# Healthcare-Robotics/mr-gan

Hardware: NVIDIA B200
Metric: gan_train_step_pairs_per_sec (higher is better)
Workload: dtype f16

## Files before the change

### mr_gan_b200/csrc/common.cuh

```cuda
#pragma once
#include <cuda_fp16.h>
#include <cuda_runtime.h>
#include <stdint.h>

#define MRGAN_TID_Z 5

enum { ACT_NONE = 0, ACT_RELU = 1, ACT_SOFTPLUS = 2, ACT_LEAKY = 3 };
enum { EPI_FWD = 0, EPI_DX = 1, EPI_STORE = 2 };

struct FoldState {
  uint32_t key0, key1;
  int iterations;
  int it_net[2];
  int rng_step;
  float lr_t[2];
  int D, n_train, n_test;
  int ldx;
  const float* x_train;
  const int* y_train;
  const int* y_test;
  const int* idx[3];
  const float* stage_x;
  const int* stage_y;
  const float* stage_z;
// ... 164 lines not shown
```

### mr_gan_b200/csrc/kernels_simt.cuh

```cuda
#pragma once
#include "common.cuh"

__device__ __forceinline__ float4 ldg4(const float* p) { return __ldg(reinterpret_cast<const float4*>(p)); }

template <bool AT, bool BT>
__global__ void __launch_bounds__(256)
k_gemm_simt(const GemmDesc* __restrict__ descs, const FoldState* __restrict__ folds, int rows_override, AdamHyper hp) {
  const GemmDesc d = descs[blockIdx.z];
  int M = d.M, K = d.K;
  const int N = d.N;
  if (rows_override > 0) { if (AT) K = rows_override; else M = rows_override; }
  const int m0 = blockIdx.y * 64, n0 = blockIdx.x * 64;
  if (m0 >= M || n0 >= N) return;

  __shared__ __align__(16) float As[2][16][68];
  __shared__ __align__(16) float Bs[2][16][68];
  const int tid = threadIdx.x, tx = tid & 15, ty = tid >> 4;
  const float4 zero4 = make_float4(0.f, 0.f, 0.f, 0.f);

  auto load_a = [&](int k0) -> float4 {
    if (AT) {
      const int k = k0 + (tid >> 4), m = m0 + (tid & 15) * 4;
      return (k < K && m < d.lda) ? ldg4(d.A + (size_t)k * d.lda + m) : zero4;
    } else {
// ... 117 lines not shown
      if (m >= M) continue;
      float v = acc[i][j];
      if (d.act == ACT_RELU) v = fmaxf(v, 0.f);
      else if (d.act == ACT_SOFTPLUS) v = softplusf(v);
      else if (d.act == ACT_LEAKY) v = v > 0.f ? v : hp.alpha * v;
      if (d.C) d.C[(size_t)m * d.ldc + n] = v;
      if (d.C2) d.C2[(size_t)m * d.ldc2 + n] = mul ? v * nz[i] : v + d.sigma * nz[i];
    }
  }
}

template <int PG>
__global__ void __launch_bounds__(128)
k_prep(FoldState* __restrict__ folds, int fold_base, int mode, int from_stage, int t, int B, int nrows,
       int noise_dim, float sigma_in, AdamHyper hp, OperandMode om) {
  FoldState& fs = folds[fold_base + blockIdx.z];
  const int c = blockIdx.x * 128 + threadIdx.x;
  const uint32_t step = (uint32_t)fs.rng_step;
  const int D = fs.D;

  if (blockIdx.x == 0 && blockIdx.y == 0) {
    if (threadIdx.x == 0) {
      const int net = (mode == 1) ? 1 : 0;
      const int tt = (hp.shared_t ? fs.iterations : fs.it_net[net]) + 1;
      const double b1t = pow((double)hp.b1, (double)tt), b2t = pow((double)hp.b2, (double)tt);
      fs.lr_t[net] = (float)((double)hp.lr * sqrt(1.0 - b2t) / (1.0 - b1t));
    }
    if (mode != 1) {
      for (int r = threadIdx.x; r < (mode == 2 ? nrows : B); r += 128)
        fs.labels_cur[r] = from_stage ? fs.stage_y[r] : fs.y_train[fs.idx[0][(size_t)t * B + r]];
// ... 154 lines not shown
  float var = 0.f;
  for (int i = 0; i < BN_SLICES; ++i) var += red[1][i][cx];
  if (!ok) return;
  const float istd = rsqrtf(var / d.B + eps);
  if (sl == 0) d.istd[j] = istd;
  const float g = d.gamma[j], b = d.beta[j];
  for (int r = sl; r < d.B; r += BN_SLICES) {
    const float xh = (d.h1[(size_t)r * d.ld + j] - mu) * istd;
    d.xhat[(size_t)r * d.ld + j] = xh;
    const float u = fmaf(g, xh, b);
    put_operand(d.u + (size_t)r * d.ldu + j, u, om);
  }
}

__global__ void __launch_bounds__(1024) k_bn_bwd(const BnDesc* __restrict__ descs, OperandMode om) {
  __shared__ float red[2][BN_MAX_SLICES][BN_COLS];
  const BnDesc d = descs[blockIdx.z];
  const int BN_SLICES = blockDim.x / BN_COLS;
  const int cx = threadIdx.x & (BN_COLS - 1), sl = threadIdx.x / BN_COLS;
  const int j = blockIdx.x * BN_COLS + cx;
  const bool ok = j < d.W;
  const float ginv = (om.mode == 2) ? 1.0f / om.gscale : 1.0f;
  float p1 = 0.f, p2 = 0.f;
  if (ok) for (int r = sl; r < d.B; r += BN_SLICES) {
    const float du = d.du[(size_t)r * d.ld + j] * ginv;
    p1 += du;
    p2 = fmaf(du, d.xhat[(size_t)r * d.ld + j], p2);
  }
  red[0][sl][cx] = p1; red[1][sl][cx] = p2;
  __syncthreads();
// ... 522 lines not shown
```

### mr_gan_b200/csrc/kernels_tc.cuh

```cuda
#pragma once
#include <cuda.h>
#include "common.cuh"

enum { HEAD_NONE = 0, HEAD_DISC = 1, HEAD_FM = 2, HEAD_BN = 3 };

struct alignas(64) TcOp {
  CUtensorMap mapA, mapB;
  GemmDesc g;
  int ME, NE, KE;
  int bn;
  int net;
  int ws_stride;
  float* ws;
  int esz;
  int head;
  int stats_stride;
  const void* hd;
  float* stats;
};

#define TC_KBLK 32
#define TC_SPIN_LIMIT (1ll << 31)

#ifdef MRGAN_PHASE_TIMING
__device__ __forceinline__ unsigned long long gtimer() { unsigned long long t; asm volatile("mov.u64 %0, %globaltimer;" : "=l"(t)); return t; }
#define PT_MARK(i) do { pt[i] = gtimer(); } while (0)
#else
#define PT_MARK(i) do { } while (0)
#endif

namespace tc {

__device__ __forceinline__ uint32_t smem_u32(const void* p) { return (uint32_t)__cvta_generic_to_shared(p); }

__device__ __forceinline__ void mbar_init(uint64_t* bar, uint32_t count) {
  asm volatile("mbarrier.init.shared::cta.b64 [%1], %0;" ::"r"(count), "r"(smem_u32(bar)) : "memory");
}
__device__ __forceinline__ void mbar_expect_tx(uint64_t* bar, uint32_t bytes) {
  asm volatile("mbarrier.arrive.expect_tx.shared::cta.b64 _, [%1], %0;" ::"r"(bytes), "r"(smem_u32(bar)) : "memory");
}
// ... 304 lines not shown
k_gemm_tc(const TcOp* __restrict__ ops, FoldState* __restrict__ folds, int rows_override, AdamHyper hp, OperandMode om) {
  using namespace tc;
#ifdef MRGAN_PHASE_TIMING
  const unsigned long long pt_t0 = gtimer();
#endif
  constexpr int KBLK = F16 ? 64 : 32;
  constexpr uint32_t MN_BOX = F16 ? 8192u : 4096u;
  const int ksplit = (B_MN && rows_override > 1) ? rows_override : 1;
  const int kslice = (int)blockIdx.z % ksplit;
  const TcOp& op = ops[blockIdx.z / ksplit];
  const int ME = op.ME, KE = op.KE, bn = op.bn;
  int NE = op.NE;
  if (rows_override > 0 && !B_MN) NE = rows_override;
  const int m0 = blockIdx.x * 128 * MT, n0 = blockIdx.y * bn;
  if (m0 >= ME || n0 >= NE) return;

  extern __shared__ uint8_t smem_raw[];
  uint8_t* smem = reinterpret_cast<uint8_t*>((reinterpret_cast<uintptr_t>(smem_raw) + 1023) & ~(uintptr_t)1023);
  const uint32_t a_bytes = MT * 128 * 128, b_bytes = (uint32_t)bn * 128, stage_bytes = a_bytes + b_bytes;
  uint64_t* bars = reinterpret_cast<uint64_t*>(smem + STAGES * stage_bytes);
  uint64_t* full = bars;
  uint64_t* empty = bars + STAGES;
  uint64_t* tmem_full = bars + 2 * STAGES;
  uint32_t* tmem_holder = reinterpret_cast<uint32_t*>(bars + 2 * STAGES + 1);
  float* const red = reinterpret_cast<float*>(bars + 24);
#ifdef MRGAN_PHASE_TIMING
  unsigned long long* pt = reinterpret_cast<unsigned long long*>(bars + 16);
  if (threadIdx.x == 0) pt[0] = pt_t0;
#endif

// ... 7 lines not shown
    prefetch_map(&op.mapA);
    prefetch_map(&op.mapB);
    for (int s = 0; s < STAGES; ++s) { mbar_init(&full[s], 1); mbar_init(&empty[s], 1); }
    mbar_init(tmem_full, 1);
    asm volatile("fence.mbarrier_init.release.cluster;" ::: "memory");
  }
  if (warp == 1) {
    asm volatile("tcgen05.alloc.cta_group::1.sync.aligned.shared::cta.b32 [%0], %1;" ::"r"(smem_u32(tmem_holder)), "r"((uint32_t)TMEM_COLS) : "memory");
    asm volatile("tcgen05.relinquish_alloc_permit.cta_group::1.sync.aligned;" ::: "memory");
  }
  fence_before();
  __syncthreads();
  fence_after();
  const uint32_t tmem_base = *tmem_holder;
  if (threadIdx.x == 0) PT_MARK(1);

  if (warp == 0) {
    if (lane == 0) {
      for (int kb = 0; kb < nkb; ++kb) {
        const int s = kb % STAGES;
        const uint32_t ph = (uint32_t)(kb / STAGES) & 1u;
        mbar_wait(&empty[s], ph ^ 1u);
        mbar_expect_tx(&full[s], stage_bytes);
        uint8_t* sa = smem + (size_t)s * stage_bytes;
        uint8_t* sb = sa + a_bytes;
        const int k0 = (kb0 + kb) * KBLK;
        if (A_MN) {
#pragma unroll
          for (int b = 0; b < (128 / KBLK) * MT; ++b) tma_load_2d(&op.mapA, &full[s], sa + b * MN_BOX, m0 + KBLK * b, k0);
        } else {
// ... 350 lines not shown
template <bool F16, int KROWS>
__global__ void __launch_bounds__(192, (TcAdamCfg<F16, KROWS>::MINB))
k_dw_adam_tc(const TcAdamOp* __restrict__ ops, FoldState* __restrict__ folds, AdamHyper hp, int nfl, int op_stride) {
  using namespace tc;
  using Cfg = TcAdamCfg<F16, KROWS>;
  constexpr int STAGES = Cfg::STAGES, KC = Cfg::KC, NB = Cfg::NB, NBUF = Cfg::NBUF;
  constexpr uint32_t STAGE_BYTES = Cfg::STAGE_BYTES, ARR_BYTES = Cfg::ARR_BYTES, CHUNK_BYTES = Cfg::CHUNK_BYTES;
  constexpr int KBLK = KROWS;
  constexpr uint32_t MN_BOX = Cfg::MN_BOX;
  constexpr int MN_BOXES = F16 ? 2 : 4;
  constexpr int MN_W = F16 ? 64 : 32;
  const TcAdamOp& op = ops[((int)blockIdx.z / nfl) * op_stride + ((int)blockIdx.z % nfl)];
  const int ME = op.ME, NE = op.NE, KE = op.KE;
  const int m0 = blockIdx.x * 128, n0 = blockIdx.y * 128;
  if (m0 >= ME || n0 >= NE) return;

  extern __shared__ __align__(1024) uint8_t smem_dyn[];
  uint8_t* smem = smem_dyn;
  if ((smem_u32(smem) & 1023u) != 0) __trap();
  uint8_t* cbuf = smem + STAGES * STAGE_BYTES;
  uint64_t* bars = reinterpret_cast<uint64_t*>(cbuf + NB * CHUNK_BYTES);
  uint64_t* full = bars;
  uint64_t* empty = bars + STAGES;
  uint64_t* tmem_full = bars + 2 * STAGES;
  uint64_t* cfull = bars + 2 * STAGES + 1;
  uint64_t* cdone = cfull + NBUF;
  uint32_t* tmem_holder = reinterpret_cast<uint32_t*>(cdone + NBUF);
  auto buf_ptr = [&](int b) -> uint8_t* { return b < NB ? cbuf + (size_t)b * CHUNK_BYTES : smem + (size_t)(b - NB) * CHUNK_BYTES; };

  const int warp = threadIdx.x >> 5, lane = threadIdx.x & 31;
// ... 5 lines not shown
    prefetch_map(&op.mapA); prefetch_map(&op.mapB); prefetch_map(&op.mapP); prefetch_map(&op.mapM); prefetch_map(&op.mapV);
    if (F16) prefetch_map(&op.mapH);
    for (int s = 0; s < STAGES; ++s) { mbar_init(&full[s], 1); mbar_init(&empty[s], 1); }
    mbar_init(tmem_full, 1);
    for (int b = 0; b < NBUF; ++b) { mbar_init(&cfull[b], 1); mbar_init(&cdone[b], 128); }
    asm volatile("fence.mbarrier_init.release.cluster;" ::: "memory");
  }
  if (warp == 1) {
    asm volatile("tcgen05.alloc.cta_group::1.sync.aligned.shared::cta.b32 [%0], %1;" ::"r"(smem_u32(tmem_holder)), "r"(128u) : "memory");
    asm volatile("tcgen05.relinquish_alloc_permit.cta_group::1.sync.aligned;" ::: "memory");
  }
  fence_before();
  __syncthreads();
  fence_after();
  const uint32_t tmem_base = *tmem_holder;

  if (warp == 0) {
    if (lane == 0) {
      auto load_chunk = [&](int c) {
        const int b = c % NBUF;
        uint8_t* dst = buf_ptr(b);
        mbar_expect_tx(&cfull[b], 3 * ARR_BYTES);
        tma_load_2d(&op.mapP, &cfull[b], dst, m0, n0 + c * KC);
        tma_load_2d(&op.mapM, &cfull[b], dst + ARR_BYTES, m0, n0 + c * KC);
        tma_load_2d(&op.mapV, &cfull[b], dst + 2 * ARR_BYTES, m0, n0 + c * KC);
      };
      for (int c = 0; c < NB && c < nch; ++c) load_chunk(c);
      for (int kb = 0; kb < nkb; ++kb) {
        const int s = kb % STAGES;
        const uint32_t ph = (uint32_t)(kb / STAGES) & 1u;
// ... 90 lines not shown
```

### mr_gan_b200/csrc/mrgan_api.cu

```cuda
#include <cuda_runtime.h>
#include <cuda_fp16.h>
#include <dlfcn.h>
#include <math.h>
#include <stdio.h>
#include <stdlib.h>
#include <string.h>
#include <algorithm>
#include <map>
#include <string>
#include <vector>

#include "../../include/mrgan.h"
#include "kernels_simt.cuh"
#include "kernels_tc.cuh"
#include "kernels_svm.cuh"
#include "kernels_dp.cuh"

namespace {

thread_local std::string g_last_error;

enum Op {
  OP_G1, OP_G2, OP_G3D, OP_G3G,
  OP_D1, OP_D2, OP_D3, OP_D4, OP_D5, OP_D6,
// ... 56 lines not shown
int tc_debug_gemm(mrgan_handle* h, int mode, const GemmDesc& g, int esz);
}

constexpr int kMaxChains = 16;
struct mrgan_handle {
  mrgan_config cfg;
  int nf = 0, R = 0, NE = 0, n_train = 0;
  std::vector<mrgan_fold_shape> shapes;
  std::vector<NetLayout> net[2];
  std::vector<FoldBuffers> fb;
  cudaStream_t stream = nullptr;
  cudaStream_t side = nullptr;
  cudaEvent_t ev_pool[16] = {nullptr}; int ev_next = 0;
  bool side_open = false;
  int nchains = 1;
  cudaStream_t cmain[kMaxChains] = {nullptr}, cside[kMaxChains] = {nullptr};
  char* arena = nullptr; size_t arena_bytes = 0;
  __half* harena = nullptr;
  OperandMode om = {0, 1.0f, nullptr, nullptr};
  float *P = nullptr, *Mo = nullptr, *Vo = nullptr, *Gr = nullptr; long long n_flat = 0;
  FoldState* d_folds = nullptr; std::vector<FoldState> h_folds;
  GemmDesc* d_descs = nullptr; std::vector<GemmDesc> h_descs;
  PermDesc* d_perm = nullptr;
  BnDesc* d_bn = nullptr; LossDesc* d_loss = nullptr; EvalDesc *d_eval = nullptr, *d_eval_s = nullptr;
  int* d_conf = nullptr;
  struct SalWork {
    char* mem = nullptr;
    GemmDesc* descs = nullptr;
    float* profile = nullptr;
    TcOp* tcops = nullptr;
// ... 326 lines not shown
  }
  CK(cudaMemcpy(h->d_descs, h->h_descs.data(), (size_t)NUM_OPS * nf * sizeof(GemmDesc), cudaMemcpyHostToDevice));
  CK(cudaMemcpy(h->d_folds, h->h_folds.data(), nf * sizeof(FoldState), cudaMemcpyHostToDevice));
  CK(cudaMemcpy(h->d_loss, ls.data(), nf * sizeof(LossDesc), cudaMemcpyHostToDevice));
  CK(cudaMemcpy(h->d_eval, ev.data(), nf * sizeof(EvalDesc), cudaMemcpyHostToDevice));
  CK(cudaMemcpy(h->d_eval_s, evs.data(), nf * sizeof(EvalDesc), cudaMemcpyHostToDevice));
  CK(cudaMemcpy(h->d_ranges[0], rg0.data(), nf * sizeof(AdamRange), cudaMemcpyHostToDevice));
  if (gan) {
    CK(cudaMemcpy(h->d_bn, bn.data(), nf * sizeof(BnDesc), cudaMemcpyHostToDevice));
    CK(cudaMemcpy(h->d_ranges[1], rg1.data(), nf * sizeof(AdamRange), cudaMemcpyHostToDevice));
  }
  return MRGAN_OK;
}

template <typename... KArgs, typename... Args>
void launch_k(mrgan_handle* h, void (*kern)(KArgs...), const cudaLaunchConfig_t& cfg, Args... args) {
  const cudaError_t e = cudaLaunchKernelEx(&cfg, kern, static_cast<KArgs>(args)...);
  if (e != cudaSuccess && !h->sticky) { h->sticky = MRGAN_ERR_CUDA; h->err = std::string("kernel launch: ") + cudaGetErrorString(e); }
  h->launches++;
}
template <typename... KArgs, typename... Args>
void launch_k(mrgan_handle* h, void (*kern)(KArgs...), dim3 grid, dim3 block, size_t smem, cudaStream_t st, Args... args) {
  cudaLaunchConfig_t cfg;
  memset(&cfg, 0, sizeof(cfg));
  cfg.gridDim = grid; cfg.blockDim = block; cfg.dynamicSmemBytes = smem; cfg.stream = st;
  launch_k(h, kern, cfg, args...);
}

void set_ones(mrgan_handle* h, float* p, int ld, int rows, int col) {
  launch_k(h, k_set_col, (rows + 127) / 128, 128, 0, h->stream, p, ld, rows, col, 1.0f, h->om);
}
// ... 560 lines not shown
      }
    }
    h->stream = origin; h->side = origin_side;
    for (int ch = 1; ch < nch; ++ch) {
      cudaEvent_t j = h->ev_pool[h->ev_next++ & 15];
      cudaEventRecord(j, h->cmain[ch]);
      cudaStreamWaitEvent(origin, j, 0);
    }
  }
  launch_k(h, k_epoch_reduce, h->nf, 32, 0, h->stream, h->d_step_stats, h->d_eval, h->d_epoch_stats, h->nf, nb,
           (int)(c.model == MRGAN_MODEL_GAN && c.eval_each_epoch));
  CK(cudaMemcpyAsync(h->h_epoch_stats, h->d_epoch_stats, (size_t)h->nf * 8 * sizeof(float), cudaMemcpyDeviceToHost, h->stream));
  CK(cudaStreamEndCapture(h->stream, &g));
  { const int sk = take_sticky(h); if (sk) { cudaGraphDestroy(g); return sk; } }
  cudaGraphExec_t ge = nullptr;
  CK(cudaGraphInstantiate(&ge, g, 0));
  CK(cudaGraphDestroy(g));
  h->graphs[key] = ge;
  h->graph_nodes[key] = h->launches - before;
  h->launches = before;
  return MRGAN_OK;
}

int upload_indices(mrgan_handle* h, const int32_t* const* streams, int n_streams, int n_idx) {
  const int slot = h->idx_slot;
  h->idx_slot ^= 1;
  CK(cudaEventSynchronize(h->idx_free[slot]));
  int* pin = h->h_idx_pinned[slot];
  for (int f = 0; f < h->nf; ++f)
    for (int s = 0; s < n_streams; ++s)
      memcpy(pin + ((size_t)f * 3 + s) * h->n_train, streams[s] + (size_t)f * n_idx, (size_t)n_idx * sizeof(int));
// ... 22 lines not shown
  cuuint64_t dims[2] = {(cuuint64_t)cols, (cuuint64_t)rows};
  cuuint64_t strides[1] = {(cuuint64_t)pitch * (cuuint64_t)esz};
  cuuint32_t box[2] = {(cuuint32_t)box_cols, (cuuint32_t)box_rows};
  cuuint32_t es[2] = {1u, 1u};
  return fn(m, esz == 2 ? CU_TENSOR_MAP_DATA_TYPE_FLOAT16 : CU_TENSOR_MAP_DATA_TYPE_FLOAT32, 2, const_cast<void*>(base), dims,
            strides, box, es, CU_TENSOR_MAP_INTERLEAVE_NONE,
            box_cols != row_elems ? CU_TENSOR_MAP_SWIZZLE_NONE
                                  : ((mn_major && esz == 4) ? CU_TENSOR_MAP_SWIZZLE_128B_ATOM_32B : CU_TENSOR_MAP_SWIZZLE_128B),
            kL2Promo,
            CU_TENSOR_MAP_FLOAT_OOB_FILL_NONE) == CUDA_SUCCESS;
}

int round_up(int x, int m) { return (x + m - 1) / m * m; }

#define TC_FWD_STAGES 4
#define TC_DW_STAGES 2
#define TC_FWD_THREADS (64 + 32 * 8)
#define TC_DW_THREADS (64 + 32 * 4)
#define K_TC_FWD(F, V) k_gemm_tc<true, false, TC_FWD_STAGES, 256, 1, 8, 1, F, V>
#define K_TC_FWD_N(F, V) k_gemm_tc<true, false, TC_FWD_STAGES, 512, 1, 8, 1, F, V>
#define K_TC_DX(F, V) k_gemm_tc<false, false, TC_FWD_STAGES, 256, 1, 8, 1, F, V>
#define K_TC_FWD2(F, V) k_gemm_tc<true, false, TC_FWD_STAGES, 512, 1, 8, 2, F, V>
#define K_TC_DX_N(F, V) k_gemm_tc<false, false, TC_FWD_STAGES, 512, 1, 8, 1, F, V>
#define K_TC_DX2(F, V) k_gemm_tc<false, false, TC_FWD_STAGES, 512, 1, 8, 2, F, V>
#define K_TC_DW(F, V) k_gemm_tc<true, true, TC_DW_STAGES, 128, 2, 4, 1, F, V>
#define TC_BIG_STAGES 3
#define K_TC_FWD_BIG(F, V) k_gemm_tc<true, false, TC_BIG_STAGES, 512, 1, 8, 2, F, V>
#define K_TC_DX_BIG(F, V) k_gemm_tc<false, false, TC_BIG_STAGES, 512, 1, 8, 2, F, V>
#define K_TC_DW_BIG(F, V) k_gemm_tc<true, true, TC_BIG_STAGES, 512, 1, 8, 2, F, V>
#define TC_LAUNCH(h, f16, K, grid, block, smem, st, ...)                          \
  do {                                                                            \
    const bool var_ = (h)->cfg.hidden_act != MRGAN_ACT_RELU || (h)->cfg.dropout > 0.0f;                \
    if (f16 && var_) launch_k(h, K(true, true), grid, block, smem, st, __VA_ARGS__);                   \
    else if (f16) launch_k(h, K(true, false), grid, block, smem, st, __VA_ARGS__);                     \
    else if (var_) launch_k(h, K(false, true), grid, block, smem, st, __VA_ARGS__);                    \
    else launch_k(h, K(false, false), grid, block, smem, st, __VA_ARGS__);                             \
  } while (0)
size_t tc_smem_bytes(int bn, int stages, int mt = 1) { return 1024 + (size_t)stages * ((size_t)mt * 128 * 128 + (size_t)bn * 128) + 256; }
bool tc_use_mt2(int maxME, int bn) { return maxME >= 500 && tc_smem_bytes(bn, TC_FWD_STAGES, 2) <= 227 * 1024; }

int tc_setup(mrgan_handle* h);

EncodeTiledFn tc_encoder() {
  EncodeTiledFn fn = nullptr;
  cudaDriverEntryPointQueryResult qres;
  if (cudaGetDriverEntryPoint("cuTensorMapEncodeTiled", (void**)&fn, cudaEnableDefault, &qres) != cudaSuccess ||
      qres != cudaDriverEntryPointSuccess) return nullptr;
  return fn;
}

template <bool F, bool V> void tc_set_smem_attr_fmt() {
  cudaFuncSetAttribute(K_TC_FWD(F, V), cudaFuncAttributeMaxDynamicSharedMemorySize, (int)tc_smem_bytes(256, TC_FWD_STAGES));
  cudaFuncSetAttribute(K_TC_FWD_N(F, V), cudaFuncAttributeMaxDynamicSharedMemorySize, (int)tc_smem_bytes(256, TC_FWD_STAGES));
  cudaFuncSetAttribute(K_TC_DX(F, V), cudaFuncAttributeMaxDynamicSharedMemorySize, (int)tc_smem_bytes(256, TC_FWD_STAGES));
  cudaFuncSetAttribute(K_TC_DX_N(F, V), cudaFuncAttributeMaxDynamicSharedMemorySize, (int)tc_smem_bytes(256, TC_FWD_STAGES));
  cudaFuncSetAttribute(K_TC_FWD_BIG(F, V), cudaFuncAttributeMaxDynamicSharedMemorySize, 227 * 1024);
  cudaFuncSetAttribute(K_TC_DX_BIG(F, V), cudaFuncAttributeMaxDynamicSharedMemorySize, 227 * 1024);
  cudaFuncSetAttribute(K_TC_DW_BIG(F, V), cudaFuncAttributeMaxDynamicSharedMemorySize, 227 * 1024);
  cudaFuncSetAttribute(K_TC_FWD2(F, V), cudaFuncAttributeMaxDynamicSharedMemorySize, 227 * 1024);
  cudaFuncSetAttribute(K_TC_DX2(F, V), cudaFuncAttributeMaxDynamicSharedMemorySize, 227 * 1024);
  cudaFuncSetAttribute(K_TC_DW(F, V), cudaFuncAttributeMaxDynamicSharedMemorySize, (int)tc_smem_bytes(128, TC_DW_STAGES));
  if (!V) cudaFuncSetAttribute(k_dw_adam_tc<F, (F ? 32 : 16)>, cudaFuncAttributeMaxDynamicSharedMemorySize, (int)TcAdamCfg<F, (F ? 32 : 16)>::SMEM);
}
void tc_set_smem_attr() {
  tc_set_smem_attr_fmt<false, false>(); tc_set_smem_attr_fmt<true, false>();
  tc_set_smem_attr_fmt<false, true>(); tc_set_smem_attr_fmt<true, true>();
}

void tc_pick_tile(int rows, int feats, int nf, int* bn, bool* mt1) {
  *bn = 256; *mt1 = false;
  auto tiles = [&](int b, bool one) { return ((feats + (one ? 127 : 255)) / (one ? 128 : 256)) * ((rows + b - 1) / b) * nf; };
  if (tiles(256, false) >= 120) return;
  *mt1 = true;
  for (int b : {256, 128, 64}) { *bn = b; if (tiles(b, true) >= 120) return; }
}

bool tc_fill_op(EncodeTiledFn fn, TcOp& t, const GemmDesc& g, int mode, int esz = 4, int bn_big = 256) {
// ... 14 lines not shown
}

int tc_debug_gemm(mrgan_handle* h, int mode, const GemmDesc& g, int esz) {
  EncodeTiledFn fn = tc_encoder();
  if (!fn) return fail(h, MRGAN_ERR_CUDA, "cuTensorMapEncodeTiled not available from the driver");
  TcOp t; memset(&t, 0, sizeof(t));
  if (!tc_fill_op(fn, t, g, mode, esz)) return fail(h, MRGAN_ERR_CUDA, "cuTensorMapEncodeTiled failed");
  Temps tmp;
  TcOp* d = nullptr;
  CK(tmp.alloc(&d, sizeof(TcOp)));
  CK(cudaMemcpyAsync(d, &t, sizeof(t), cudaMemcpyHostToDevice, h->stream));
  tc_set_smem_attr();
  dim3 grid((t.ME + 127) / 128, (t.NE + t.bn - 1) / t.bn, 1);
  const OperandMode om0{0, 1.0f, nullptr, nullptr};
  const bool f16 = esz == 2;
  if (mode == 0) TC_LAUNCH(h, f16, K_TC_FWD, grid, dim3(TC_FWD_THREADS), tc_smem_bytes(t.bn, TC_FWD_STAGES), h->stream, (const TcOp*)d, h->d_folds, 0, h->hp, om0);
  else if (mode == 1) TC_LAUNCH(h, f16, K_TC_DX, grid, dim3(TC_FWD_THREADS), tc_smem_bytes(t.bn, TC_FWD_STAGES), h->stream, (const TcOp*)d, h->d_folds, 0, h->hp, om0);
  else TC_LAUNCH(h, f16, K_TC_DW, grid, dim3(TC_DW_THREADS), tc_smem_bytes(t.bn, TC_DW_STAGES), h->stream, (const TcOp*)d, h->d_folds, 0, h->hp, om0);
  CK(cudaStreamSynchronize(h->stream));
  return MRGAN_OK;
}

int tc_make_op(mrgan_handle* h, EncodeTiledFn fn, int op, TcOp* ts) {
  const OpInfo& oi = h->ops[op];
  if (!oi.used) return MRGAN_OK;
  const int nf = h->nf;
  for (int f = 0; f < nf; ++f) {
    const GemmDesc& g = h->h_descs[(size_t)op * nf + f];
    TcOp& t = ts[f];
    const int mode = (!oi.at && !oi.bt) ? 0 : ((!oi.at && oi.bt) ? 1 : 2);
    int bn_big = 256;
    if (mode != 2 && oi.maxM > 256) { bool m1; tc_pick_tile(oi.maxM, oi.maxN, nf, &bn_big, &m1); h->tc_mt1[op] = m1; }
    if (h->om.mode == 2) {
// ... 135 lines not shown
  for (int n = 0; n < 2; ++n) { if (h->d_ranges_tc[n]) cudaFree(h->d_ranges_tc[n]); h->d_ranges_tc[n] = nullptr; }
  for (int i = 0; i < NUM_OPS; ++i) { h->tc_bn[i] = 0; h->tc_maxME[i] = 0; h->tc_maxNE[i] = 0; h->tc_mt1[i] = false; }
  h->d_tcadam = nullptr;
  h->d_tcops = nullptr;
}

void tc_launch_dw_adam(mrgan_handle* h, int op, int nlayers, int f0, int nfl, cudaStream_t st) {
  const bool f16 = h->om.mode == 2;
  int gx = 0, gy = 0;
  for (int l = 0; l < nlayers; ++l) {
    gx = std::max(gx, (h->tc_maxME[op + l] + 127) / 128);
    gy = std::max(gy, (h->tc_maxNE[op + l] + 127) / 128);
  }
  const dim3 grid(gx, gy, nlayers * nfl);
  const TcAdamOp* ad = h->d_tcadam + (size_t)op * h->nf + f0;
  if (f16) launch_k(h, k_dw_adam_tc<true, 32>, grid, dim3(192), TcAdamCfg<true, 32>::SMEM, st, ad, h->d_folds, h->hp, nfl, h->nf);
  else launch_k(h, k_dw_adam_tc<false, 16>, grid, dim3(192), TcAdamCfg<false, 16>::SMEM, st, ad, h->d_folds, h->hp, nfl, h->nf);
}

bool tc_dw_merge(const mrgan_handle* h) { return h->cfg.precision != MRGAN_PREC_FP32 && h->d_tcadam != nullptr; }

bool tc_launch_gemm(mrgan_handle* h, int op, int f0, int nfl, int rows_override, cudaStream_t st) {
  const OpInfo& oi = h->ops[op];
  const bool f16 = h->om.mode == 2;
  const int bn = h->tc_bn[op];
  int NE = h->tc_maxNE[op];
  if (rows_override > 0 && !oi.at) NE = rows_override;
  dim3 grid((h->tc_maxME[op] + 127) / 128, (NE + bn - 1) / bn, nfl);
  const TcOp* d = (op < NUM_OPS ? h->d_tcops + (size_t)op * h->nf : h->sal.tcops + (size_t)(op - NUM_OPS) * h->nf) + f0;
  if (bn == 256 && (oi.at || h->tc_maxME[op] >= 500) && !h->tc_mt1[op]) {
    grid.x = (h->tc_maxME[op] + 255) / 256;
    const size_t smem = tc_smem_bytes(256, TC_BIG_STAGES, 2);
    if (oi.at) {
      const int ks = h->tc_ksplit[op] > 1 ? h->tc_ksplit[op] : 1;
      grid.z = nfl * ks;
      TC_LAUNCH(h, f16, K_TC_DW_BIG, grid, dim3(TC_FWD_THREADS), smem, st, d, h->d_folds, ks, h->hp, h->om);
      if (ks > 1) {
        const int n4 = h->tc_maxNE[op] * pitch8(h->tc_maxME[op]) / 4;
        launch_k(h, k_splitk_reduce, dim3(std::min((n4 + 255) / 256, 1184), nfl, 1), dim3(256), 0, st, d, ks);
      }
    } else if (!oi.bt) TC_LAUNCH(h, f16, K_TC_FWD_BIG, grid, dim3(TC_FWD_THREADS), smem, st, d, h->d_folds, rows_override, h->hp, h->om);
    else TC_LAUNCH(h, f16, K_TC_DX_BIG, grid, dim3(TC_FWD_THREADS), smem, st, d, h->d_folds, rows_override, h->hp, h->om);
    return true;
  }
  const bool head_mt2 = (h->tc_heads & 2) && op == OP_D5G;
  if (!oi.at && !h->tc_mt1[op] && (tc_use_mt2(h->tc_maxME[op], bn) || head_mt2)) {
    grid.x = (h->tc_maxME[op] + 255) / 256;
    const size_t smem = tc_smem_bytes(bn, TC_FWD_STAGES, 2);
    if (!oi.bt) TC_LAUNCH(h, f16, K_TC_FWD2, grid, dim3(TC_FWD_THREADS), smem, st, d, h->d_folds, rows_override, h->hp, h->om);
    else TC_LAUNCH(h, f16, K_TC_DX2, grid, dim3(TC_FWD_THREADS), smem, st, d, h->d_folds, rows_override, h->hp, h->om);
    return true;
  }
  if (!oi.at && !oi.bt) {
    if (2 * tc_smem_bytes(bn, TC_FWD_STAGES) > 227 * 1024)
      TC_LAUNCH(h, f16, K_TC_FWD_N, grid, dim3(TC_FWD_THREADS), tc_smem_bytes(bn, TC_FWD_STAGES), st, d, h->d_folds, rows_override, h->hp, h->om);
    else
      TC_LAUNCH(h, f16, K_TC_FWD, grid, dim3(TC_FWD_THREADS), tc_smem_bytes(bn, TC_FWD_STAGES), st, d, h->d_folds, rows_override, h->hp, h->om);
  }
  else if (!oi.at && oi.bt) {
    if (2 * tc_smem_bytes(bn, TC_FWD_STAGES) > 227 * 1024)
      TC_LAUNCH(h, f16, K_TC_DX_N, grid, dim3(TC_FWD_THREADS), tc_smem_bytes(bn, TC_FWD_STAGES), st, d, h->d_folds, rows_override, h->hp, h->om);
    else
      TC_LAUNCH(h, f16, K_TC_DX, grid, dim3(TC_FWD_THREADS), tc_smem_bytes(bn, TC_FWD_STAGES), st, d, h->d_folds, rows_override, h->hp, h->om);
  }
  else if (h->d_tcadam) { tc_launch_dw_adam(h, op, 1, f0, nfl, st); return true; }
  else TC_LAUNCH(h, f16, K_TC_DW, grid, dim3(TC_DW_THREADS), tc_smem_bytes(bn, TC_DW_STAGES), st, d, h->d_folds, 0, h->hp, h->om);
  return true;
}

}

extern "C" {

const char* mrgan_version(void) { return "mrgan-b200 0.2 (sm_100a)"; }

int mrgan_abi_info(int out[4]) {
  if (!out) return fail(nullptr, MRGAN_ERR_ARG, "abi_info: null pointer");
  out[0] = MRGAN_ABI_VERSION; out[1] = (int)sizeof(mrgan_config); out[2] = (int)sizeof(mrgan_fold_shape); out[3] = (int)sizeof(mrgan_epoch_stats);
  return MRGAN_OK;
}

// ... 93 lines not shown
  ok = ok && cudaStreamCreateWithFlags(&h->side, cudaStreamNonBlocking) == cudaSuccess;
  for (int i = 0; i < 16 && ok; ++i) ok = cudaEventCreateWithFlags(&h->ev_pool[i], cudaEventDisableTiming) == cudaSuccess;
  {
    const char* env = getenv("MRGAN_CHAINS");
    int nch = env ? atoi(env) : (h->nf >= 32 ? 4 : (h->nf >= 8 ? 2 : 1));
    if (nch < 1) nch = 1;
    if (nch > kMaxChains) nch = kMaxChains;
    if (nch > h->nf) nch = h->nf;
    h->nchains = nch;
    h->cmain[0] = h->stream; h->cside[0] = h->side;
    for (int ch = 1; ch < nch && ok; ++ch) {
      ok = cudaStreamCreateWithFlags(&h->cmain[ch], cudaStreamNonBlocking) == cudaSuccess &&
           cudaStreamCreateWithFlags(&h->cside[ch], cudaStreamNonBlocking) == cudaSuccess;
    }
  }
  ok = ok && cudaEventCreate(&h->ev0) == cudaSuccess && cudaEventCreate(&h->ev1) == cudaSuccess;
  ok = ok && cudaMallocHost(&h->h_epoch_stats, (size_t)h->nf * 8 * sizeof(float)) == cudaSuccess;
  ok = ok && cudaMallocHost(&h->h_scratch, 64 * sizeof(float)) == cudaSuccess;
  for (int s = 0; s < 2 && ok; ++s) {
    ok = ok && cudaMallocHost(&h->h_idx_pinned[s], (size_t)h->nf * 3 * h->n_train * sizeof(int)) == cudaSuccess;
    ok = ok && cudaEventCreateWithFlags(&h->idx_free[s], cudaEventDisableTiming) == cudaSuccess;
  }
  if (!ok) return cleanup(fail(nullptr, MRGAN_ERR_CUDA, "stream/event/pinned allocation failed"));
  if (cfg->model != MRGAN_MODEL_SVM) {
    const int rc = build_descs(h); if (rc != MRGAN_OK) return cleanup(rc);
    init_ones(h);
  } else {
    std::vector<EvalDesc> ev(h->nf);
    for (int f = 0; f < h->nf; ++f) ev[f] = EvalDesc{nullptr, 0, h->fb[f].yte, folds[f].n_test, 0, nullptr, h->fb[f].pred};
    if (cudaMemcpy(h->d_eval, ev.data(), h->nf * sizeof(EvalDesc), cudaMemcpyHostToDevice) != cudaSuccess)
// ... 410 lines not shown
  CK(cudaMemcpyAsync(dm, m, n * 4, cudaMemcpyHostToDevice, h->stream));
  CK(cudaMemcpyAsync(dv, v, n * 4, cudaMemcpyHostToDevice, h->stream));
  CK(cudaMemcpyAsync(dg, g, n * 4, cudaMemcpyHostToDevice, h->stream));
  const double b1t = pow((double)h->hp.b1, (double)t), b2t = pow((double)h->hp.b2, (double)t);
  const float lr_t = (float)((double)h->hp.lr * sqrt(1.0 - b2t) / (1.0 - b1t));
  int blocks = (int)((n4 + 255) / 256); if (blocks > 4096) blocks = 4096;
  launch_k(h, k_adam_plain, blocks, 256, 0, h->stream, (float4*)dp, (float4*)dm, (float4*)dv, (const float4*)dg, n4, lr_t,
           h->hp.b1, h->hp.b2, h->hp.eps);
  CK(cudaMemcpyAsync(p, dp, n * 4, cudaMemcpyDeviceToHost, h->stream));
  CK(cudaMemcpyAsync(m, dm, n * 4, cudaMemcpyDeviceToHost, h->stream));
  CK(cudaMemcpyAsync(v, dv, n * 4, cudaMemcpyDeviceToHost, h->stream));
  return complete(h);
}

static void svm_launch(mrgan_handle* h, int phase);

int mrgan_time_op(mrgan_handle* h, int which, int reps, float* ms_avg) {
  TRY(enter(h, "time_op", 0));
  if (!ms_avg || reps < 1) return fail(h, MRGAN_ERR_ARG, "time_op: bad argument");
  const bool svm = h->cfg.model == MRGAN_MODEL_SVM, gan = h->cfg.model == MRGAN_MODEL_GAN;
  if (svm != (which >= MRGAN_TIME_SVM_KMAT && which <= MRGAN_TIME_SVM_PREDICT))
    return fail(h, which < 0 || which > MRGAN_TIME_SALIENCY ? MRGAN_ERR_ARG : MRGAN_ERR_STATE, "time_op: op does not exist for this model");
  if (which < 0 || which > MRGAN_TIME_SALIENCY) return fail(h, MRGAN_ERR_ARG, "time_op: unknown op");
  if (!gan && (which == MRGAN_TIME_ADAM_G || which == MRGAN_TIME_GEN_STEP || which == MRGAN_TIME_DX1)) return fail(h, MRGAN_ERR_STATE, "time_op: no generator in this model");
  TRY(ready(h, "time_op", svm ? FITTED : (LOADED | (which == MRGAN_TIME_SALIENCY ? LOCAL : 0u))));
  if (svm) return time_reps(h, reps, [&]() { svm_launch(h, which); }, ms_avg);
  if (which == MRGAN_TIME_SALIENCY) TRY(saliency_setup(h));
  return time_reps(h, reps, [&]() {
    switch (which) {
      case MRGAN_TIME_ADAM_D: launch_adam(h, 0, h->nf, 0); break;
// ... 202 lines not shown
  std::vector<TcOp> ops(groups);
  memset(ops.data(), 0, sizeof(TcOp) * groups);
  for (int g = 0; g < groups; ++g) {
    float* A = buf + (sa + sb + sc) * g; float* B = A + sa; float* C = B + sb;
    GemmDesc d = make_desc(A, lda, B, ldb, C, ldc, M, N, K, mode == 0 ? EPI_FWD : (mode == 1 ? EPI_DX : EPI_STORE), ACT_NONE, 0);
    if (!tc_fill_op(fn, ops[g], d, mode)) return fail(h, MRGAN_ERR_CUDA, "cuTensorMapEncodeTiled failed");
  }
  TcOp* dops = nullptr;
  CK(tmp.alloc(&dops, sizeof(TcOp) * groups));
  CK(cudaMemcpyAsync(dops, ops.data(), sizeof(TcOp) * groups, cudaMemcpyHostToDevice, h->stream));
  tc_set_smem_attr();
  const TcOp& t = ops[0];
  const dim3 grid((t.ME + 127) / 128, (t.NE + t.bn - 1) / t.bn, groups);
  const OperandMode om0{0, 1.0f, nullptr, nullptr};
  return time_reps(h, reps, [&]() {
    if (mode == 0) launch_k(h, K_TC_FWD(false, false), grid, TC_FWD_THREADS, tc_smem_bytes(t.bn, TC_FWD_STAGES), h->stream, dops, h->d_folds, 0, h->hp, om0);
    else if (mode == 1) launch_k(h, K_TC_DX(false, false), grid, TC_FWD_THREADS, tc_smem_bytes(t.bn, TC_FWD_STAGES), h->stream, dops, h->d_folds, 0, h->hp, om0);
    else launch_k(h, K_TC_DW(false, false), grid, TC_DW_THREADS, tc_smem_bytes(t.bn, TC_DW_STAGES), h->stream, dops, h->d_folds, 0, h->hp, om0);
  }, ms);
}


static void svm_launch(mrgan_handle* h, int phase) {
  mrgan_handle::Svm& S = h->svm;
  const int nf = h->nf;
  if (phase == MRGAN_TIME_SVM_KMAT) {
    launch_k(h, k_svm_split, dim3((S.max_rows + 7) / 8, 2 * nf), 256, 0, h->stream, S.d_split);
    launch_k(h, k_svm_kmat, dim3((S.n_lab + SVM_BM - 1) / SVM_BM, (S.max_rows + SVM_BN - 1) / SVM_BN, 2 * nf), SVM_KMAT_THREADS,
             SVM_KMAT_SMEM, h->stream, S.d_gemm);
  } else if (phase == MRGAN_TIME_SVM_SMO) {
    launch_k(h, k_svm_smo, nf * S.npairs, SVM_SMO_THREADS, (size_t)SVM_SMO_SMEM_PER_ROW * S.npmax, h->stream, S.d_jobs, S.eps);
  } else {
    launch_k(h, k_svm_vote, dim3(S.max_nte, nf), SVM_VOTE_THREADS, 0, h->stream, S.d_jobs, S.npairs, h->cfg.n_classes, S.d_Kt, nullptr,
// ... 453 lines not shown
```

Baseline: 43960.

## Budget TMEM via smem floors, drop 512-col variants, add launch priorities

Removes the 512-TMEM-column FWD_N/DX_N kernel variants and always uses the 256-column kernels. A per-kernel minimum dynamic shared memory request caps how many tcgen05 CTAs can share an SM, and a compile-time check proves no such set can exceed 512 TMEM columns, so TMEM allocation never has to wait. Every launch now carries a priority attribute (high on the main stream, low on the side stream) and graphs are instantiated to honour node priority. A residency tracing hook is added behind a timing macro; the cost is lower occupancy for small-smem GEMMs.

```diff
diff --git a/mr_gan_b200/csrc/common.cuh b/mr_gan_b200/csrc/common.cuh
--- a/mr_gan_b200/csrc/common.cuh
+++ b/mr_gan_b200/csrc/common.cuh
@@ -4,6 +4,34 @@
 #include <stdint.h>
 
 #define MRGAN_TID_Z 5
+
+#ifdef MRGAN_PHASE_TIMING
+__device__ __forceinline__ unsigned long long gtimer() { unsigned long long t; asm volatile("mov.u64 %0, %%globaltimer;" : "=l"(t)); return t; }
+
+enum { RES_FWD = 0, RES_DX = 1, RES_DW = 2, RES_DW_ADAM = 3, RES_PREP = 4, RES_BN_BWD = 5 };
+struct ResRec { unsigned long long t_entry, t_alloc, t_exit; unsigned smid, cls, op, pad; };
+__device__ ResRec* g_res;
+__device__ unsigned g_res_cap, g_res_n;
+struct ResScope {
+  unsigned long long t0, t1;
+  unsigned cls, op;
+  __device__ ResScope(unsigned c, unsigned o) : cls(c), op(o) { t0 = t1 = gtimer(); }
+  __device__ void alloced() { t1 = gtimer(); }
+  __device__ ~ResScope() {
+    if (threadIdx.x != 0 || !g_res) return;
+    const unsigned i = atomicAdd(&g_res_n, 1u);
+    if (i >= g_res_cap) return;
+    unsigned sm;
+    asm volatile("mov.u32 %0, %%smid;" : "=r"(sm));
+    g_res[i] = ResRec{t0, t1, gtimer(), sm, cls, op, 0u};
+  }
+};
+#define RES_SCOPE(c, o) ResScope res_scope_((c), (o))
+#define RES_ALLOCED() res_scope_.alloced()
+#else
+#define RES_SCOPE(c, o) do { } while (0)
+#define RES_ALLOCED() do { } while (0)
+#endif
 
 enum { ACT_NONE = 0, ACT_RELU = 1, ACT_SOFTPLUS = 2, ACT_LEAKY = 3 };
 enum { EPI_FWD = 0, EPI_DX = 1, EPI_STORE = 2 };
diff --git a/mr_gan_b200/csrc/kernels_simt.cuh b/mr_gan_b200/csrc/kernels_simt.cuh
--- a/mr_gan_b200/csrc/kernels_simt.cuh
+++ b/mr_gan_b200/csrc/kernels_simt.cuh
@@ -155,6 +155,7 @@
 __global__ void __launch_bounds__(128)
 k_prep(FoldState* __restrict__ folds, int fold_base, int mode, int from_stage, int t, int B, int nrows,
        int noise_dim, float sigma_in, AdamHyper hp, OperandMode om) {
+  RES_SCOPE(RES_PREP, (unsigned)mode);
   FoldState& fs = folds[fold_base + blockIdx.z];
   const int c = blockIdx.x * 128 + threadIdx.x;
   const uint32_t step = (uint32_t)fs.rng_step;
@@ -339,6 +340,7 @@
 }
 
 __global__ void __launch_bounds__(1024) k_bn_bwd(const BnDesc* __restrict__ descs, OperandMode om) {
+  RES_SCOPE(RES_BN_BWD, 0u);
   __shared__ float red[2][BN_MAX_SLICES][BN_COLS];
   const BnDesc d = descs[blockIdx.z];
   const int BN_SLICES = blockDim.x / BN_COLS;
diff --git a/mr_gan_b200/csrc/kernels_tc.cuh b/mr_gan_b200/csrc/kernels_tc.cuh
--- a/mr_gan_b200/csrc/kernels_tc.cuh
+++ b/mr_gan_b200/csrc/kernels_tc.cuh
@@ -23,7 +23,6 @@
 #define TC_SPIN_LIMIT (1ll << 31)
 
 #ifdef MRGAN_PHASE_TIMING
-__device__ __forceinline__ unsigned long long gtimer() { unsigned long long t; asm volatile("mov.u64 %0, %globaltimer;" : "=l"(t)); return t; }
 #define PT_MARK(i) do { pt[i] = gtimer(); } while (0)
 #else
 #define PT_MARK(i) do { } while (0)
@@ -358,6 +357,7 @@
   if (rows_override > 0 && !B_MN) NE = rows_override;
   const int m0 = blockIdx.x * 128 * MT, n0 = blockIdx.y * bn;
   if (m0 >= ME || n0 >= NE) return;
+  RES_SCOPE((B_MN ? RES_DW : (A_MN ? RES_FWD : RES_DX)) | (MT << 4) | (STAGES << 8) | (TMEM_COLS << 16), ((unsigned)KE << 16) | (unsigned)ME);
 
   extern __shared__ uint8_t smem_raw[];
   uint8_t* smem = reinterpret_cast<uint8_t*>((reinterpret_cast<uintptr_t>(smem_raw) + 1023) & ~(uintptr_t)1023);
@@ -395,6 +395,7 @@
   fence_after();
   const uint32_t tmem_base = *tmem_holder;
   if (threadIdx.x == 0) PT_MARK(1);
+  RES_ALLOCED();
 
   if (warp == 0) {
     if (lane == 0) {
@@ -775,6 +776,7 @@
   const int ME = op.ME, NE = op.NE, KE = op.KE;
   const int m0 = blockIdx.x * 128, n0 = blockIdx.y * 128;
   if (m0 >= ME || n0 >= NE) return;
+  RES_SCOPE(RES_DW_ADAM | (1 << 4) | (STAGES << 8) | (128 << 16), ((unsigned)KE << 16) | (unsigned)ME);
 
   extern __shared__ __align__(1024) uint8_t smem_dyn[];
   uint8_t* smem = smem_dyn;
@@ -810,6 +812,7 @@
   __syncthreads();
   fence_after();
   const uint32_t tmem_base = *tmem_holder;
+  RES_ALLOCED();
 
   if (warp == 0) {
     if (lane == 0) {
diff --git a/mr_gan_b200/csrc/mrgan_api.cu b/mr_gan_b200/csrc/mrgan_api.cu
--- a/mr_gan_b200/csrc/mrgan_api.cu
+++ b/mr_gan_b200/csrc/mrgan_api.cu
@@ -94,6 +94,7 @@
   cudaEvent_t ev_pool[16] = {nullptr}; int ev_next = 0;
   bool side_open = false;
   int nchains = 1;
+  int prio_hi = 0, prio_lo = 0;
   cudaStream_t cmain[kMaxChains] = {nullptr}, cside[kMaxChains] = {nullptr};
   char* arena = nullptr; size_t arena_bytes = 0;
   __half* harena = nullptr;
@@ -450,7 +451,14 @@
 }
 
 template <typename... KArgs, typename... Args>
-void launch_k(mrgan_handle* h, void (*kern)(KArgs...), const cudaLaunchConfig_t& cfg, Args... args) {
+void launch_k(mrgan_handle* h, void (*kern)(KArgs...), const cudaLaunchConfig_t& cfg0, Args... args) {
+  cudaLaunchConfig_t cfg = cfg0;
+  cudaLaunchAttribute attrs[4];
+  unsigned n = 0;
+  for (; n < cfg0.numAttrs && n < 3; ++n) attrs[n] = cfg0.attrs[n];
+  attrs[n].id = cudaLaunchAttributePriority;
+  attrs[n].val.priority = cfg0.stream == h->side ? h->prio_lo : h->prio_hi;
+  cfg.attrs = attrs; cfg.numAttrs = n + 1;
   const cudaError_t e = cudaLaunchKernelEx(&cfg, kern, static_cast<KArgs>(args)...);
   if (e != cudaSuccess && !h->sticky) { h->sticky = MRGAN_ERR_CUDA; h->err = std::string("kernel launch: ") + cudaGetErrorString(e); }
   h->launches++;
@@ -1041,7 +1049,7 @@
   CK(cudaStreamEndCapture(h->stream, &g));
   { const int sk = take_sticky(h); if (sk) { cudaGraphDestroy(g); return sk; } }
   cudaGraphExec_t ge = nullptr;
-  CK(cudaGraphInstantiate(&ge, g, 0));
+  CK(cudaGraphInstantiate(&ge, g, cudaGraphInstantiateFlagUseNodePriority));
   CK(cudaGraphDestroy(g));
   h->graphs[key] = ge;
   h->graph_nodes[key] = h->launches - before;
@@ -1094,14 +1102,13 @@
 int round_up(int x, int m) { return (x + m - 1) / m * m; }
 
 #define TC_FWD_STAGES 4
+#define TC_N_STAGES 4
 #define TC_DW_STAGES 2
 #define TC_FWD_THREADS (64 + 32 * 8)
 #define TC_DW_THREADS (64 + 32 * 4)
-#define K_TC_FWD(F, V) k_gemm_tc<true, false, TC_FWD_STAGES, 256, 1, 8, 1, F, V>
-#define K_TC_FWD_N(F, V) k_gemm_tc<true, false, TC_FWD_STAGES, 512, 1, 8, 1, F, V>
-#define K_TC_DX(F, V) k_gemm_tc<false, false, TC_FWD_STAGES, 256, 1, 8, 1, F, V>
+#define K_TC_FWD(F, V) k_gemm_tc<true, false, TC_N_STAGES, 256, 1, 8, 1, F, V>
+#define K_TC_DX(F, V) k_gemm_tc<false, false, TC_N_STAGES, 256, 1, 8, 1, F, V>
 #define K_TC_FWD2(F, V) k_gemm_tc<true, false, TC_FWD_STAGES, 512, 1, 8, 2, F, V>
-#define K_TC_DX_N(F, V) k_gemm_tc<false, false, TC_FWD_STAGES, 512, 1, 8, 1, F, V>
 #define K_TC_DX2(F, V) k_gemm_tc<false, false, TC_FWD_STAGES, 512, 1, 8, 2, F, V>
 #define K_TC_DW(F, V) k_gemm_tc<true, true, TC_DW_STAGES, 128, 2, 4, 1, F, V>
 #define TC_BIG_STAGES 3
@@ -1116,8 +1123,35 @@
     else if (var_) launch_k(h, K(false, true), grid, block, smem, st, __VA_ARGS__);                    \
     else launch_k(h, K(false, false), grid, block, smem, st, __VA_ARGS__);                             \
   } while (0)
-size_t tc_smem_bytes(int bn, int stages, int mt = 1) { return 1024 + (size_t)stages * ((size_t)mt * 128 * 128 + (size_t)bn * 128) + 256; }
+constexpr size_t tc_smem_bytes(int bn, int stages, int mt = 1) { return 1024 + (size_t)stages * ((size_t)mt * 128 * 128 + (size_t)bn * 128) + 256; }
 bool tc_use_mt2(int maxME, int bn) { return maxME >= 500 && tc_smem_bytes(bn, TC_FWD_STAGES, 2) <= 227 * 1024; }
+
+constexpr size_t TC_N_SMEM_MIN = 76 * 1024;
+size_t tc_n_smem(int bn) { return std::max(tc_smem_bytes(bn, TC_N_STAGES), TC_N_SMEM_MIN); }
+constexpr size_t TC_MT2_SMEM_MIN = 153 * 1024;
+size_t tc_mt2_smem(int bn) { return std::max(tc_smem_bytes(bn, TC_FWD_STAGES, 2), TC_MT2_SMEM_MIN); }
+constexpr size_t TC_DW_SMEM_MIN = 74 * 1024;
+size_t tc_dw_smem(int bn) { return std::max(tc_smem_bytes(bn, TC_DW_STAGES), TC_DW_SMEM_MIN); }
+constexpr size_t TC_ADAM_SMEM = TcAdamCfg<true, 32>::SMEM;
+static_assert(TcAdamCfg<false, 16>::SMEM <= TC_ADAM_SMEM, "k_dw_adam_tc<false, 16> outgrew the shared memory it requests");
+struct TcBudget { size_t smem; int cols; };
+constexpr TcBudget kTcBudget[] = {
+    {TC_N_SMEM_MIN, 256},
+    {TC_MT2_SMEM_MIN, 512},
+    {TC_ADAM_SMEM, 128},
+    {TC_DW_SMEM_MIN, 128},
+    {227 * 1024, 512},
+};
+constexpr int kTcBudgetN = (int)(sizeof(kTcBudget) / sizeof(kTcBudget[0]));
+constexpr bool tc_budget_ok(int j = 0, size_t smem = 0, int cols = 0) {
+  if (cols > 512) return false;
+  for (int k = j; k < kTcBudgetN; ++k) {
+    const size_t s = smem + kTcBudget[k].smem + 1024;
+    if (s <= 228 * 1024 && !tc_budget_ok(k, s, cols + kTcBudget[k].cols)) return false;
+  }
+  return true;
+}
+static_assert(tc_budget_ok(), "a set of tcgen05 CTAs that fits an SM's shared memory would exceed its 512 TMEM columns");
 
 int tc_setup(mrgan_handle* h);
 
@@ -1130,17 +1164,15 @@
 }
 
 template <bool F, bool V> void tc_set_smem_attr_fmt() {
-  cudaFuncSetAttribute(K_TC_FWD(F, V), cudaFuncAttributeMaxDynamicSharedMemorySize, (int)tc_smem_bytes(256, TC_FWD_STAGES));
-  cudaFuncSetAttribute(K_TC_FWD_N(F, V), cudaFuncAttributeMaxDynamicSharedMemorySize, (int)tc_smem_bytes(256, TC_FWD_STAGES));
-  cudaFuncSetAttribute(K_TC_DX(F, V), cudaFuncAttributeMaxDynamicSharedMemorySize, (int)tc_smem_bytes(256, TC_FWD_STAGES));
-  cudaFuncSetAttribute(K_TC_DX_N(F, V), cudaFuncAttributeMaxDynamicSharedMemorySize, (int)tc_smem_bytes(256, TC_FWD_STAGES));
+  cudaFuncSetAttribute(K_TC_FWD(F, V), cudaFuncAttributeMaxDynamicSharedMemorySize, (int)tc_n_smem(256));
+  cudaFuncSetAttribute(K_TC_DX(F, V), cudaFuncAttributeMaxDynamicSharedMemorySize, (int)tc_n_smem(256));
   cudaFuncSetAttribute(K_TC_FWD_BIG(F, V), cudaFuncAttributeMaxDynamicSharedMemorySize, 227 * 1024);
   cudaFuncSetAttribute(K_TC_DX_BIG(F, V), cudaFuncAttributeMaxDynamicSharedMemorySize, 227 * 1024);
   cudaFuncSetAttribute(K_TC_DW_BIG(F, V), cudaFuncAttributeMaxDynamicSharedMemorySize, 227 * 1024);
   cudaFuncSetAttribute(K_TC_FWD2(F, V), cudaFuncAttributeMaxDynamicSharedMemorySize, 227 * 1024);
   cudaFuncSetAttribute(K_TC_DX2(F, V), cudaFuncAttributeMaxDynamicSharedMemorySize, 227 * 1024);
-  cudaFuncSetAttribute(K_TC_DW(F, V), cudaFuncAttributeMaxDynamicSharedMemorySize, (int)tc_smem_bytes(128, TC_DW_STAGES));
-  if (!V) cudaFuncSetAttribute(k_dw_adam_tc<F, (F ? 32 : 16)>, cudaFuncAttributeMaxDynamicSharedMemorySize, (int)TcAdamCfg<F, (F ? 32 : 16)>::SMEM);
+  cudaFuncSetAttribute(K_TC_DW(F, V), cudaFuncAttributeMaxDynamicSharedMemorySize, (int)tc_dw_smem(256));
+  if (!V) cudaFuncSetAttribute(k_dw_adam_tc<F, (F ? 32 : 16)>, cudaFuncAttributeMaxDynamicSharedMemorySize, (int)TC_ADAM_SMEM);
 }
 void tc_set_smem_attr() {
   tc_set_smem_attr_fmt<false, false>(); tc_set_smem_attr_fmt<true, false>();
@@ -1185,9 +1217,9 @@
   dim3 grid((t.ME + 127) / 128, (t.NE + t.bn - 1) / t.bn, 1);
   const OperandMode om0{0, 1.0f, nullptr, nullptr};
   const bool f16 = esz == 2;
-  if (mode == 0) TC_LAUNCH(h, f16, K_TC_FWD, grid, dim3(TC_FWD_THREADS), tc_smem_bytes(t.bn, TC_FWD_STAGES), h->stream, (const TcOp*)d, h->d_folds, 0, h->hp, om0);
-  else if (mode == 1) TC_LAUNCH(h, f16, K_TC_DX, grid, dim3(TC_FWD_THREADS), tc_smem_bytes(t.bn, TC_FWD_STAGES), h->stream, (const TcOp*)d, h->d_folds, 0, h->hp, om0);
-  else TC_LAUNCH(h, f16, K_TC_DW, grid, dim3(TC_DW_THREADS), tc_smem_bytes(t.bn, TC_DW_STAGES), h->stream, (const TcOp*)d, h->d_folds, 0, h->hp, om0);
+  if (mode == 0) TC_LAUNCH(h, f16, K_TC_FWD, grid, dim3(TC_FWD_THREADS), tc_n_smem(t.bn), h->stream, (const TcOp*)d, h->d_folds, 0, h->hp, om0);
+  else if (mode == 1) TC_LAUNCH(h, f16, K_TC_DX, grid, dim3(TC_FWD_THREADS), tc_n_smem(t.bn), h->stream, (const TcOp*)d, h->d_folds, 0, h->hp, om0);
+  else TC_LAUNCH(h, f16, K_TC_DW, grid, dim3(TC_DW_THREADS), tc_dw_smem(t.bn), h->stream, (const TcOp*)d, h->d_folds, 0, h->hp, om0);
   CK(cudaStreamSynchronize(h->stream));
   return MRGAN_OK;
 }
@@ -1353,8 +1385,8 @@
   }
   const dim3 grid(gx, gy, nlayers * nfl);
   const TcAdamOp* ad = h->d_tcadam + (size_t)op * h->nf + f0;
-  if (f16) launch_k(h, k_dw_adam_tc<true, 32>, grid, dim3(192), TcAdamCfg<true, 32>::SMEM, st, ad, h->d_folds, h->hp, nfl, h->nf);
-  else launch_k(h, k_dw_adam_tc<false, 16>, grid, dim3(192), TcAdamCfg<false, 16>::SMEM, st, ad, h->d_folds, h->hp, nfl, h->nf);
+  if (f16) launch_k(h, k_dw_adam_tc<true, 32>, grid, dim3(192), TC_ADAM_SMEM, st, ad, h->d_folds, h->hp, nfl, h->nf);
+  else launch_k(h, k_dw_adam_tc<false, 16>, grid, dim3(192), TC_ADAM_SMEM, st, ad, h->d_folds, h->hp, nfl, h->nf);
 }
 
 bool tc_dw_merge(const mrgan_handle* h) { return h->cfg.precision != MRGAN_PREC_FP32 && h->d_tcadam != nullptr; }
@@ -1385,25 +1417,17 @@
   const bool head_mt2 = (h->tc_heads & 2) && op == OP_D5G;
   if (!oi.at && !h->tc_mt1[op] && (tc_use_mt2(h->tc_maxME[op], bn) || head_mt2)) {
     grid.x = (h->tc_maxME[op] + 255) / 256;
-    const size_t smem = tc_smem_bytes(bn, TC_FWD_STAGES, 2);
+    const size_t smem = tc_mt2_smem(bn);
     if (!oi.bt) TC_LAUNCH(h, f16, K_TC_FWD2, grid, dim3(TC_FWD_THREADS), smem, st, d, h->d_folds, rows_override, h->hp, h->om);
     else TC_LAUNCH(h, f16, K_TC_DX2, grid, dim3(TC_FWD_THREADS), smem, st, d, h->d_folds, rows_override, h->hp, h->om);
     return true;
   }
-  if (!oi.at && !oi.bt) {
-    if (2 * tc_smem_bytes(bn, TC_FWD_STAGES) > 227 * 1024)
-      TC_LAUNCH(h, f16, K_TC_FWD_N, grid, dim3(TC_FWD_THREADS), tc_smem_bytes(bn, TC_FWD_STAGES), st, d, h->d_folds, rows_override, h->hp, h->om);
-    else
-      TC_LAUNCH(h, f16, K_TC_FWD, grid, dim3(TC_FWD_THREADS), tc_smem_bytes(bn, TC_FWD_STAGES), st, d, h->d_folds, rows_override, h->hp, h->om);
-  }
-  else if (!oi.at && oi.bt) {
-    if (2 * tc_smem_bytes(bn, TC_FWD_STAGES) > 227 * 1024)
-      TC_LAUNCH(h, f16, K_TC_DX_N, grid, dim3(TC_FWD_THREADS), tc_smem_bytes(bn, TC_FWD_STAGES), st, d, h->d_folds, rows_override, h->hp, h->om);
-    else
-      TC_LAUNCH(h, f16, K_TC_DX, grid, dim3(TC_FWD_THREADS), tc_smem_bytes(bn, TC_FWD_STAGES), st, d, h->d_folds, rows_override, h->hp, h->om);
-  }
+  if (!oi.at && !oi.bt)
+    TC_LAUNCH(h, f16, K_TC_FWD, grid, dim3(TC_FWD_THREADS), tc_n_smem(bn), st, d, h->d_folds, rows_override, h->hp, h->om);
+  else if (!oi.at && oi.bt)
+    TC_LAUNCH(h, f16, K_TC_DX, grid, dim3(TC_FWD_THREADS), tc_n_smem(bn), st, d, h->d_folds, rows_override, h->hp, h->om);
   else if (h->d_tcadam) { tc_launch_dw_adam(h, op, 1, f0, nfl, st); return true; }
-  else TC_LAUNCH(h, f16, K_TC_DW, grid, dim3(TC_DW_THREADS), tc_smem_bytes(bn, TC_DW_STAGES), st, d, h->d_folds, 0, h->hp, h->om);
+  else TC_LAUNCH(h, f16, K_TC_DW, grid, dim3(TC_DW_THREADS), tc_dw_smem(bn), st, d, h->d_folds, 0, h->hp, h->om);
   return true;
 }
 
@@ -1527,6 +1551,7 @@
            cudaStreamCreateWithFlags(&h->cside[ch], cudaStreamNonBlocking) == cudaSuccess;
     }
   }
+  ok = ok && cudaDeviceGetStreamPriorityRange(&h->prio_lo, &h->prio_hi) == cudaSuccess;
   ok = ok && cudaEventCreate(&h->ev0) == cudaSuccess && cudaEventCreate(&h->ev1) == cudaSuccess;
   ok = ok && cudaMallocHost(&h->h_epoch_stats, (size_t)h->nf * 8 * sizeof(float)) == cudaSuccess;
   ok = ok && cudaMallocHost(&h->h_scratch, 64 * sizeof(float)) == cudaSuccess;
@@ -1967,6 +1992,30 @@
 }
 
 static void svm_launch(mrgan_handle* h, int phase);
+
+#ifdef MRGAN_PHASE_TIMING
+static ResRec* g_res_host_buf = nullptr;
+int mrgan_trace_arm(mrgan_handle* h, unsigned cap) {
+  TRY(enter(h, "trace_arm", 0));
+  CK(cudaDeviceSynchronize());
+  if (g_res_host_buf) { cudaFree(g_res_host_buf); g_res_host_buf = nullptr; }
+  if (cap) CK(cudaMalloc(&g_res_host_buf, (size_t)cap * sizeof(ResRec)));
+  const unsigned zero = 0;
+  CK(cudaMemcpyToSymbol(g_res, &g_res_host_buf, sizeof(ResRec*)));
+  CK(cudaMemcpyToSymbol(g_res_cap, &cap, sizeof(unsigned)));
+  CK(cudaMemcpyToSymbol(g_res_n, &zero, sizeof(unsigned)));
+  return MRGAN_OK;
+}
+int mrgan_trace_read(mrgan_handle* h, void* out, unsigned cap, unsigned* n) {
+  TRY(enter(h, "trace_read", 0));
+  if (!out || !n) return fail(h, MRGAN_ERR_ARG, "trace_read: null pointer");
+  CK(cudaDeviceSynchronize());
+  CK(cudaMemcpyFromSymbol(n, g_res_n, sizeof(unsigned)));
+  const unsigned k = std::min(*n, cap);
+  if (k) CK(cudaMemcpy(out, g_res_host_buf, (size_t)k * sizeof(ResRec), cudaMemcpyDeviceToHost));
+  return MRGAN_OK;
+}
+#endif
 
 int mrgan_time_op(mrgan_handle* h, int which, int reps, float* ms_avg) {
   TRY(enter(h, "time_op", 0));
@@ -2199,9 +2248,9 @@
   const dim3 grid((t.ME + 127) / 128, (t.NE + t.bn - 1) / t.bn, groups);
   const OperandMode om0{0, 1.0f, nullptr, nullptr};
   return time_reps(h, reps, [&]() {
-    if (mode == 0) launch_k(h, K_TC_FWD(false, false), grid, TC_FWD_THREADS, tc_smem_bytes(t.bn, TC_FWD_STAGES), h->stream, dops, h->d_folds, 0, h->hp, om0);
-    else if (mode == 1) launch_k(h, K_TC_DX(false, false), grid, TC_FWD_THREADS, tc_smem_bytes(t.bn, TC_FWD_STAGES), h->stream, dops, h->d_folds, 0, h->hp, om0);
-    else launch_k(h, K_TC_DW(false, false), grid, TC_DW_THREADS, tc_smem_bytes(t.bn, TC_DW_STAGES), h->stream, dops, h->d_folds, 0, h->hp, om0);
+    if (mode == 0) launch_k(h, K_TC_FWD(false, false), grid, TC_FWD_THREADS, tc_n_smem(t.bn), h->stream, dops, h->d_folds, 0, h->hp, om0);
+    else if (mode == 1) launch_k(h, K_TC_DX(false, false), grid, TC_FWD_THREADS, tc_n_smem(t.bn), h->stream, dops, h->d_folds, 0, h->hp, om0);
+    else launch_k(h, K_TC_DW(false, false), grid, TC_DW_THREADS, tc_dw_smem(t.bn), h->stream, dops, h->d_folds, 0, h->hp, om0);
   }, ms);
 }
 
```

After: 43530 (median of 6 runs). -1.0%, worse.
